# vedant-jumle/reinforcement-learning-101

Hardware: AMD Instinct MI355X
Metric: env-steps/sec (whole node), N parallel drones, 1/2/4/8 MI355X; HBM GB/s %peak (higher is better)
Workload: dtype f64

## Files before the change

reinforcement-learning-101_amd/csrc/frame.h:

```cpp
#pragma once

#include <hip/hip_runtime.h>
#include <stdint.h>
#include <string.h>

#include <type_traits>

#include "dronestep.h"
#include "philox.h"
#include "trig.h"

#include "libm_tables.h"
__device__ const double dd_libm_pow_tab[384] = DD_LIBM_POW_TAB;
__device__ const uint64_t dd_libm_exp_tab[256] = DD_LIBM_EXP_TAB;
__device__ const double dd_libm_sincos_tab[440] = DD_LIBM_SINCOS_TAB;
#define DD_LIBM_FN __device__ __forceinline__
#define DD_LIBM_OPAQUE
#define DD_LIBM_ENTRY __device__ __forceinline__
#include "libm_ref.h"
#undef DD_LIBM_FN
#undef DD_LIBM_ENTRY
#undef DD_LIBM_SINCOS_FN
#undef DD_LIBM_OPAQUE

namespace dd {

constexpr double kDeg2Rad = 3.14159265358979323846 / 180.0;

template <bool kExact = false, bool kSgpr = false>
__device__ __forceinline__ void sincos_deg(double deg, double* s, double* c) {
    if constexpr (kExact) {
        libm::sincos(deg * kDeg2Rad, s, c);
        return;
    }
    trig::sincos<kSgpr>(deg * kDeg2Rad, s, c);
}

constexpr DDConfig reference_config() {
    DDConfig c{};
    c.gravity = 0.3;
    c.drag = 0.99;
    c.angular_drag = 0.95;
    c.main_thrust_power = 0.6;
    c.side_thrust_power = 0.3;
    c.fuel_main = 2.0;
    c.fuel_side = 1.0;
    c.max_fuel = 1000.0;
    c.drone_half_height = 20 / 2.0;
    c.dt = 1.0;
    c.platform_half_width = 100 / 2.0;
    c.platform_half_height = 20 / 2.0;
    c.platform_speed = 1.0;
    c.platform_min_x = 100 / 2;
    c.platform_max_x = 800 - 100 / 2;
    c.max_landing_velocity = 3.0;
    c.max_landing_angle = 20.0;
    c.world_width = 800;
    c.world_height = 600;
    c.oob_margin = 50;
    c.ground_level = 600 - 50;
    c.wind_x = 0.0;
    c.wind_y = 0.0;
    c.reward_step = -0.1;
    c.reward_landing = 100.0;
    c.reward_crash = -100.0;
    c.reward_out_of_fuel = -50.0;
    c.reward_out_of_bounds = -50.0;
    c.shaping_offset = 500;
    c.shaping_scale = 5000;
    c.vel_scale = 10.0;
    c.angle_scale = 180.0;
    c.drone_start_x = 800 / 2;
    c.drone_start_y = 100;
    c.drone_x_min = 100;
    c.drone_x_max = 700;
    c.drone_y_min = 50;
    c.drone_y_max = 250;
    c.platform_start_x = 800 / 2;
    c.platform_start_y = 600 - 100;
    c.platform_x_lo = 100 / 2 + 50;
    c.platform_x_hi = 800 - 100 / 2 - 50;
    c.platform_y_lo = 100;
    c.platform_y_hi = 550;
    c.wind_enabled = 0;
    c.platform_moving = 0;
    c.randomize_drone = 0;
    c.randomize_platform = 1;
    c.auto_reset = 0;
    c.seed = 0;
    return c;
}

struct Consts {
    DDConfig c;
    double inv_w, inv_h, inv_vel, inv_angle, inv_fuel, inv_shaping;
};

constexpr Consts make_consts(const DDConfig& c) {
    Consts k{};
    k.c = c;
    k.inv_w = 1.0 / c.world_width;
    k.inv_h = 1.0 / c.world_height;
    k.inv_vel = 1.0 / c.vel_scale;
    k.inv_angle = 1.0 / c.angle_scale;
    k.inv_fuel = 1.0 / c.max_fuel;
    k.inv_shaping = 1.0 / c.shaping_scale;
    return k;
}

__device__ constexpr Consts kRefConsts = make_consts(reference_config());

inline bool uses_reference_physics(const DDConfig& c) {
    if (c.wind_enabled || c.platform_moving) return false;
    const DDConfig r = reference_config();
    const double* a = &c.gravity;
    const double* b = &r.gravity;
    const int n = (int)((&c.angle_scale - &c.gravity) + 1);
    for (int j = 0; j < n; ++j) {
        if (a + j == &c.wind_x || a + j == &c.wind_y) continue;
        if (memcmp(a + j, b + j, sizeof(double)) != 0) return false;
    }
    return true;
}

__device__ __forceinline__ int32_t draw_range(uint32_t r, int32_t lo, uint32_t span) {
    return lo + (int32_t)(((uint64_t)r * span) >> 32);
}

struct Lane {
    double x, y, vx, vy, angle, omega, fuel, px, py, total;
    double speed, dist;
    uint32_t status;
    int32_t steps, episode;
};

template <bool kUnscaled = false>
__device__ __forceinline__ double measure(Lane& s) {
    const double dx = s.px - s.x, dy = s.py - s.y;
    const double ss = s.vx * s.vx + s.vy * s.vy;
    const double dd = dx * dx + dy * dy;
    if (!kUnscaled) {
        s.speed = sqrt(ss);
        s.dist = sqrt(dd);
        return ss;
    }
    if (__builtin_expect(__ballot(!(ss >= 0x1p-767) | !(dd >= 0x1p-767)) != 0, 0)) {
        s.speed = sqrt(ss);
        s.dist = sqrt(dd);
    } else {
        s.speed = trig::sqrt_unscaled(ss);
        s.dist = trig::sqrt_unscaled(dd);
    }
    return ss;
}

__device__ __forceinline__ void spawn_words(const DDConfig& c, int64_t env, int32_t episode, uint32_t (&r)[4]) {
    philox4x32_7((uint32_t)env, (uint32_t)((uint64_t)env >> 32), (uint32_t)episode, 0u, (uint32_t)c.seed,
                  (uint32_t)(c.seed >> 32), r);
}

template <bool kRandom = false>
__device__ __forceinline__ void spawn_from(const DDConfig& c, double max_fuel, const uint32_t (&r)[4], Lane& s) {
    if (kRandom || c.randomize_drone) {
        s.x = draw_range(r[0], c.drone_x_min, (uint32_t)(c.drone_x_max - c.drone_x_min + 1));
        s.y = draw_range(r[1], c.drone_y_min, (uint32_t)(c.drone_y_max - c.drone_y_min + 1));
    } else {
        s.x = c.drone_start_x;
        s.y = c.drone_start_y;
    }
    if (kRandom || c.randomize_platform) {
        s.px = draw_range(r[2], c.platform_x_lo, (uint32_t)(c.platform_x_hi - c.platform_x_lo));
        s.py = draw_range(r[3], c.platform_y_lo, (uint32_t)(c.platform_y_hi - c.platform_y_lo));
    } else {
        s.px = c.platform_start_x;
        s.py = c.platform_start_y;
    }
    s.vx = 0.0; s.vy = 0.0; s.angle = 0.0; s.omega = 0.0;
    s.fuel = max_fuel;
    s.status = 0u;
    s.steps = 0;
    s.total = 0.0;
    const double dx = s.px - s.x, dy = s.py - s.y;
    s.speed = 0.0;
    s.dist = trig::sqrt_unscaled(dx * dx + dy * dy);
}

template <bool kRandom = false>
__device__ __forceinline__ void spawn(const DDConfig& c, double max_fuel, int64_t env, Lane& s) {
    s.episode += 1;
    uint32_t r[4];
    spawn_words(c, env, s.episode, r);
    spawn_from<kRandom>(c, max_fuel, r, s);
}

struct SpawnAhead {
    uint32_t r[4];
    int32_t ep;
    static constexpr int kRefill = 32;

    __device__ __forceinline__ void init(const DDConfig& c, int64_t env, int32_t episode) {
        ep = episode + 1;
        spawn_words(c, env, ep, r);
    }
    __device__ __forceinline__ void refill(const DDConfig& c, int64_t env, int32_t episode, int f) {
        if ((f & (kRefill - 1)) == kRefill - 1) {
            const bool spent = ep != episode + 1;
            if (__ballot(spent)) {
                if (spent) init(c, env, episode);
            }
        }
    }
    __device__ __forceinline__ void respawn(const DDConfig& c, double max_fuel, int64_t env, Lane& s) {
        s.episode += 1;
        uint32_t w[4] = {r[0], r[1], r[2], r[3]};
        if (ep != s.episode) spawn_words(c, env, s.episode, w);
        spawn_from(c, max_fuel, w, s);
    }
};

__device__ __forceinline__ double wrap_angle(double a) {
    double w = a > 180.0 ? a - 360.0 : a;
    w = a < -180.0 ? a + 360.0 : w;
    if (__builtin_expect(fabs(a) > 540.0, 0)) {
        w = trig::normalize_angle(a);
    }
    return w;
}

struct ThrustTrig {
    double s, c;
};
__device__ __forceinline__ void next_trig(const Lane& s, ThrustTrig& t) { sincos_deg<false>(s.angle, &t.s, &t.c); }

template <bool kRef, bool kFlat, bool kExact = false, bool kDefer = false, bool kPipe = false>
__device__ __forceinline__ double frame(const Consts& k, const DDConfig& sw, uint32_t act, Lane& s, bool* risky_out,
                                        const ThrustTrig* tt = nullptr) {
    static_assert(!kPipe || (kFlat && !kExact), "the pipelined thrust trig is the loops' fast frame");
    static_assert(!kDefer || (kRef && kFlat && !kExact), "deferred frames: reference world, rollout form");
    const DDConfig& c = k.c;

    const double ty = -c.main_thrust_power;
    constexpr bool kSgpr = !kFlat;
    const auto thrust = [&](double sa, double ca, double* dvx, double* dvy) __attribute__((always_inline)) {
        if constexpr (kRef) {
            *dvx = c.main_thrust_power * sa + 0.0;
            *dvy = ty * ca;
        } else {
            *dvx = 0.0 * ca - ty * sa;
            *dvy = 0.0 * sa + ty * ca;
        }
    };
    const bool main_on = (act & 1u) && s.fuel > 0.0;
    if constexpr (kFlat) {
        double sa, ca, dvx, dvy;
        if constexpr (kPipe) {
            sa = tt->s;
            ca = tt->c;
        } else {
            sincos_deg<kExact>(s.angle, &sa, &ca);
        }
        thrust(sa, ca, &dvx, &dvy);
        s.vx = main_on ? s.vx + dvx : s.vx;
        s.vy = main_on ? s.vy + dvy : s.vy;
        s.fuel = main_on ? s.fuel - c.fuel_main : s.fuel;
        const bool left_on = (act & 2u) && s.fuel > 0.0;
        s.omega = left_on ? s.omega - c.side_thrust_power : s.omega;
        s.fuel = left_on ? s.fuel - c.fuel_side : s.fuel;
        const bool right_on = (act & 4u) && s.fuel > 0.0;
        s.omega = right_on ? s.omega + c.side_thrust_power : s.omega;
        s.fuel = right_on ? s.fuel - c.fuel_side : s.fuel;
    } else {
        if (main_on) {
            double sa, ca, dvx, dvy;
            sincos_deg<kExact, kSgpr>(s.angle, &sa, &ca);
            thrust(sa, ca, &dvx, &dvy);
            s.vx += dvx;
            s.vy += dvy;
            s.fuel -= c.fuel_main;
        }
        if ((act & 2u) && s.fuel > 0.0) { s.omega -= c.side_thrust_power; s.fuel -= c.fuel_side; }
        if ((act & 4u) && s.fuel > 0.0) { s.omega += c.side_thrust_power; s.fuel -= c.fuel_side; }
    }
    s.fuel = s.fuel > 0.0 ? s.fuel : 0.0;

    if (!kRef && sw.wind_enabled) { s.vx += sw.wind_x; s.vy += sw.wind_y; }

    s.vy += c.gravity * c.dt;
    s.vx *= c.drag;
    s.vy *= c.drag;
    s.x += s.vx * c.dt;
    s.y += s.vy * c.dt;
    s.angle += s.omega * c.dt;
    s.omega *= c.angular_drag;
    s.angle = kFlat ? wrap_angle(s.angle) : trig::normalize_angle(s.angle);

    if (!kRef && sw.platform_moving) {
        const double dir = (s.status & DD_ST_PLAT_LEFT) ? -1.0 : 1.0;
        s.px += c.platform_speed * dir * c.dt;
        if (s.px <= c.platform_min_x) { s.px = c.platform_min_x; s.status &= ~DD_ST_PLAT_LEFT; }
        else if (s.px >= c.platform_max_x) { s.px = c.platform_max_x; s.status |= DD_ST_PLAT_LEFT; }
    }

    const auto close = [](double q, double b) { return fabs(q - b) <= 0x1p-20 * (1.0 + fabs(b)); };
    bool risky = false;
    if constexpr (!kExact) {
        if constexpr (kRef) {
            constexpr DDConfig r = reference_config();
            static_assert(-r.oob_margin == -50 && r.world_width + r.oob_margin == 850 && r.ground_level == 550,
                          "float boundary constants");
            const float xf = (float)s.x, yf = (float)s.y;
            const float qx = fabsf(fabsf(xf - 400.0f) - 450.0f), qy = fabsf(fabsf(yf - 250.0f) - 300.0f);
            risky = fminf(qx, qy) == 0.0f;
        } else {
            const bool q0 = close(s.y, c.ground_level), q1 = close(s.x, -c.oob_margin),
                       q2 = close(s.x, c.world_width + c.oob_margin), q3 = close(s.y, -c.oob_margin),
                       q4 = close(s.y, c.world_height + c.oob_margin);
            risky = q0 | q1 | q2 | q3 | q4;
        }
    }

    const double ss = kDefer ? s.vx * s.vx + s.vy * s.vy : measure<!kFlat>(s);
    const bool upright = fabs(s.angle) <= c.max_landing_angle;
    bool on_pad = false;
    const double rx = c.platform_half_width + fabs(c.drone_half_height);
    const double ry = c.platform_half_height + fabs(c.drone_half_height);
    const bool near_pad = upright && fma(-fabs(s.x), 0x1p-30, fabs(s.x - s.px)) <= rx + 1.0 &&
                          fma(-fabs(s.y), 0x1p-30, fabs(s.y - s.py)) <= ry + 1.0;
    if constexpr (kRef && !kExact) {
        const bool edge = fabs(ss - 9.0) <= 0x1p-20;
        static_assert(reference_config().max_landing_velocity == 3.0, "the squared speed limit");
        const bool slow = kDefer ? !(ss > 9.0) : !(s.speed > c.max_landing_velocity);
        risky |= near_pad & edge;
        const bool pad_test = near_pad & slow;
        if ((kFlat && !kDefer) || pad_test) {
            static_assert(reference_config().max_landing_angle == 20.0 &&
                              reference_config().drone_half_height == 10.0 &&
                              reference_config().platform_half_width == 50.0 &&
                              reference_config().platform_half_height == 10.0,
                          "sincos_upright_deg's range; the pad's half extents");
            double sb, cb;
            trig::sincos_upright_deg<kSgpr>(s.angle, &sb, &cb);
            const double bx = s.x - c.drone_half_height * sb;
            const double by = s.y + c.drone_half_height * cb;
            const double dxp = bx - s.px, dyp = by - s.py;
            const bool in_x = fabs(dxp) <= c.platform_half_width, in_y = fabs(dyp) <= c.platform_half_height;
            const bool in_box = in_x & in_y;
            const double m = fmin(fabs(fabs(dxp) - c.platform_half_width), fabs(fabs(dyp) - c.platform_half_height));
            const bool band = m <= 0x1p-19 * (1.0 + fabs(bx) + fabs(by));
            on_pad = pad_test && in_box;
            risky |= pad_test && band;
        }
    } else if (near_pad) {
        const bool edge = kRef ? fabs(ss - 9.0) <= 0x1p-20 : close(s.speed, c.max_landing_velocity);
        bool slow = !(s.speed > c.max_landing_velocity);
        if constexpr (kExact) {
            if (edge) {
                double sq = 0.0, v = s.vx;
#pragma unroll 1
                for (int q = 0; q < 2; ++q) {
                    sq += libm::pow2(v);
                    v = s.vy;
                }
                slow = !(sqrt(sq) > c.max_landing_velocity);
            }
        } else {
            risky |= edge;
        }
        if (slow) {
            double sb, cb;
            sincos_deg<kExact, kSgpr>(s.angle, &sb, &cb);
            const double bx = s.x + (0.0 * cb - c.drone_half_height * sb);
            const double by = s.y + (0.0 * sb + c.drone_half_height * cb);
            on_pad = (s.px - c.platform_half_width <= bx) & (bx <= s.px + c.platform_half_width) &
                     (s.py - c.platform_half_height <= by) & (by <= s.py + c.platform_half_height);
            if constexpr (!kExact) {
                const double m = fmin(fmin(fabs(bx - (s.px - c.platform_half_width)),
                                           fabs(bx - (s.px + c.platform_half_width))),
                                      fmin(fabs(by - (s.py - c.platform_half_height)),
                                           fabs(by - (s.py + c.platform_half_height))));
                risky |= m <= 0x1p-19 * (1.0 + fabs(bx) + fabs(by));
            }
        }
    }
    if constexpr (!kExact) *risky_out = risky;

    const bool landing = on_pad;
    const bool crash = s.y > c.ground_level;
    const bool no_fuel = s.fuel <= 0.0;
    const bool oob = (s.x < -c.oob_margin) | (s.x > c.world_width + c.oob_margin) |
                     (s.y < -c.oob_margin) | (s.y > c.world_height + c.oob_margin);
    double term = trig::div_exact(c.shaping_offset - s.dist, c.shaping_scale, k.inv_shaping);
    const bool terminal = landing | crash | no_fuel | oob;
    if constexpr (kRef) {
        constexpr DDConfig r = reference_config();
        static_assert(r.reward_landing == 100.0 && r.reward_crash == -100.0 && r.reward_out_of_fuel == -50.0 &&
                      r.reward_out_of_bounds == -50.0, "integer terminal rewards");
        const int32_t ti = landing ? 100 : crash ? -100 : -50;
        term = terminal ? (double)ti : term;
    } else {
        term = oob ? c.reward_out_of_bounds : term;
        term = no_fuel ? c.reward_out_of_fuel : term;
        term = crash ? c.reward_crash : term;
        term = landing ? c.reward_landing : term;
    }
    s.status |= landing ? (DD_ST_LANDED | DD_ST_DONE) : terminal ? (DD_ST_CRASHED | DD_ST_DONE) : 0u;
    if constexpr (kDefer) {
        s.steps += 1;
        return 0.0;
    }
    const double reward = c.reward_step + term;
    s.total += reward;
    s.steps += 1;
    return reward;
}



template <typename T>
__device__ __forceinline__ double finish_deferred(Lane& s, bool was_done, bool auto_reset, double& total) {
    constexpr DDConfig r = reference_config();
    const double dx = s.px - s.x, dy = s.py - s.y;
    s.speed = sqrt(s.vx * s.vx + s.vy * s.vy);
    s.dist = sqrt(dx * dx + dy * dy);
    if (was_done) {
        total = auto_reset ? 0.0 : total;
        return 0.0;
    }
    const bool terminal = (s.status & DD_ST_DONE) != 0;
    const int32_t ti = (s.status & DD_ST_LANDED) ? 100 : s.y > r.ground_level ? -100 : -50;
    double term = trig::div_exact(r.shaping_offset - s.dist, r.shaping_scale, kRefConsts.inv_shaping);
    term = terminal ? (double)ti : term;
    const double reward = r.reward_step + term;
    total = (double)(T)(total + reward);
    return reward;
}

template <bool kRef, bool kFlat, bool kDefer = false, bool kPipe = false, typename TQ = double>
__device__ __forceinline__ double frame_checked(const Consts& k, const DDConfig& sw, uint32_t act, Lane& s,
                                                ThrustTrig* tt = nullptr) {
    const Lane s0 = s;
    bool risky = false;
    double reward = frame<kRef, kFlat, false, kDefer, kPipe>(k, sw, act, s, &risky, tt);
    if constexpr (kPipe) sincos_deg<false>((double)(TQ)s.angle, &tt->s, &tt->c);
    if (__builtin_expect(__ballot(risky) != 0, 0)) {
        if (risky) {
            s = s0;
            reward = frame<kRef, false, true>(k, sw, act, s, nullptr);
        }
    }
    return reward;
}

template <bool kGuard = false, bool kExactDiv = false>
__device__ __forceinline__ void observe_values(const Consts& k, const Lane& s, double v[13]) {
    const DDConfig& c = k.c;
    const double dx = s.px - s.x, dy = s.py - s.y;
#define DD_Q(x, d, inv) \
    (!kExactDiv ? (x) * (inv) : kGuard ? trig::div_exact_guarded((x), (d), (inv)) : trig::div_exact((x), (d), (inv)))
    v[0] = DD_Q(s.x, c.world_width, k.inv_w);
    v[1] = DD_Q(s.y, c.world_height, k.inv_h);
    v[2] = DD_Q(s.vx, c.vel_scale, k.inv_vel);
    v[3] = DD_Q(s.vy, c.vel_scale, k.inv_vel);
    v[4] = DD_Q(s.angle, c.angle_scale, k.inv_angle);
    v[5] = DD_Q(s.omega, c.vel_scale, k.inv_vel);
    v[6] = DD_Q(s.fuel, c.max_fuel, k.inv_fuel);
    v[7] = DD_Q(s.px, c.world_width, k.inv_w);
    v[8] = DD_Q(s.py, c.world_height, k.inv_h);
    v[9] = DD_Q(s.dist, c.world_width, k.inv_w);
    v[10] = DD_Q(dx, c.world_width, k.inv_w);
    v[11] = DD_Q(dy, c.world_height, k.inv_h);
    v[12] = DD_Q(s.speed, c.vel_scale, k.inv_vel);
#undef DD_Q
}

__device__ __forceinline__ void write_obs_row(const double v[13], uint32_t status, float* o) {
#pragma unroll
    for (int j = 0; j < 13; ++j) o[j] = (float)v[j];
    o[13] = (status & DD_ST_LANDED) ? 1.0f : 0.0f;
    o[14] = (status & DD_ST_CRASHED) ? 1.0f : 0.0f;
}

template <bool kGuard = false>
__device__ __forceinline__ void observe(const Consts& k, const Lane& s, float* o) {
    double v[13];
    observe_values<kGuard>(k, s, v);
    write_obs_row(v, s.status, o);
}

enum { kShapeNone = 0, kShapePpo = 1, kShapeReinforce = 2 };

__device__ __forceinline__ double notebook_reward(const double v[13], uint32_t status, double prev_dist) {
    const double vx = v[2], vy = v[3], angle = v[4], fuel = v[6], dist = v[9], dx = v[10], dy = v[11],
                 speed = v[12];
    const bool have_prev = !__builtin_isnan(prev_dist);
    const double delta = prev_dist - dist;
    const double vtp = dist > 1e-6 ? (vx * dx + vy * dy) / dist : 0.0;
    const bool fast_toward = (speed >= 0.15) & (vtp > 0.1) & (dist > 0.065);
    const double clipped = fmin(fmax(delta * 1000 * (1.0 + speed * 2.0), -2.0), 5.0);
    const bool away = !fast_toward & (delta < -0.001);
    double distance = fast_toward ? clipped : away ? -2.0 * fabs(delta) * 1000 : 0.0;
    double hovering = (fast_toward | away) ? 0.0 : speed < 0.05 ? -1.0 : speed < 0.15 ? -0.3 : 0.0;
    distance = have_prev ? distance : 0.0;
    hovering = have_prev ? hovering : 0.0;
    double total = 0.0;
    total += -0.5;
    total += distance;
    total += hovering;
    const double excess = fabs(angle) - (((0.20 - 0.111) * dist) + 0.111);
    total += -(excess > 0.0 ? excess : 0.0);
    const double over = dist < 1 ? speed - 0.1 : speed - 0.6;
    total += (dist < 1 ? -2.0 : -1.0) * (over > 0.0 ? over : 0.0);
    total += dy > 0.0 ? 0.0 : dy * 4.0;
    const bool landed = status & DD_ST_LANDED, crashed = status & DD_ST_CRASHED;
    const double crash_term = dist > 0.3 ? -200.0 - 100.0 : -200.0;
    total += landed ? 800.0 + fuel * 100.0 : crashed ? crash_term : 0.0;
    return total;
}

__device__ __forceinline__ double reinforce_reward(const double v[13], uint32_t status) {
    const double vx = v[2], vy = v[3], angle = v[4], fuel = v[6], dist = v[9], dx = v[10], dy = v[11],
                 speed = v[12];
    constexpr double kScale = 1.0 - 0.3;
    const double time_penalty = -(kScale * (1.0 / (1.0 + (50.0 * (dist * dist))))) - 0.3;
    const double odx0 = -dx, ody0 = -dy;
    const double onorm = sqrt(odx0 * odx0 + ody0 * ody0);
    const double odx = odx0 / onorm, ody = ody0 / onorm;
    const double align_v = (vx / speed) * odx + (vy / speed) * ody;
    const double align = onorm < 1e-6 ? 1.0 : speed < 1e-6 ? 0.0 : align_v;
    const bool above = (dist > 0.065) & (dy > 0.0);
    const double sig = 4.5 * (1.0 / (1.0 + exp(10.0 * (dist - 0.5))));
    const double distance = above ? ((align > 0.0 ? 1.0 : 0.0) * speed) * sig : 0.0;
    const double valign = (above & (align > 0.0)) ? 0.5 : 0.0;
    double total = time_penalty;
    total += distance;
    total += valign;
    const double excess = fabs(angle) - (((0.20 - 0.111) * dist) + 0.111);
    total += -(excess > 0.0 ? excess : 0.0);
    const double over = dist < 1 ? speed - 0.1 : speed - 0.4;
    total += (dist < 1 ? -2.0 : -1.0) * (over > 0.0 ? over : 0.0);
    total += dy > 0.0 ? 0.0 : dy * 4.0;
    const bool landed = status & DD_ST_LANDED, crashed = status & DD_ST_CRASHED;
    const double crash_term = dist > 0.3 ? -200.0 - 100.0 : -200.0;
    total += landed ? 500.0 + fuel * 100.0 : crashed ? crash_term : 0.0;
    return total;
}

__device__ __forceinline__ void notebook_reward_parts(const double v[13], uint32_t status, double prev_dist,
                                                      double parts[8]) {
    const double vx = v[2], vy = v[3], angle = v[4], fuel = v[6], dist = v[9], dx = v[10], dy = v[11],
                 speed = v[12];
    parts[0] = -(1.0 * (1.0 / (1.0 + (100.0 * (dist * dist))))) - 0.0;
    const bool have_prev = !__builtin_isnan(prev_dist);
    const double delta = prev_dist - dist;
    const double vtp = dist > 1e-6 ? (vx * dx + vy * dy) / dist : 0.0;
    const bool fast_toward = (speed >= 0.15) & (vtp > 0.1) & (dist > 0.065);
    const double clipped = fmin(fmax(delta * 1000 * (1.0 + speed * 2.0), -2.0), 5.0);
    const bool away = !fast_toward & (delta < -0.001);
    double distance = fast_toward ? clipped : away ? -2.0 * fabs(delta) * 1000 : 0.0;
    double hovering = (fast_toward | away) ? 0.0 : speed < 0.05 ? -1.0 : speed < 0.15 ? -0.3 : 0.0;
    parts[1] = have_prev ? distance : 0.0;
    parts[2] = have_prev ? hovering : 0.0;
    const double excess = fabs(angle) - (((0.20 - 0.111) * dist) + 0.111);
    parts[3] = -(excess > 0.0 ? excess : 0.0);
    const double over = dist < 1 ? speed - 0.1 : speed - 0.6;
    parts[4] = (dist < 1 ? -2.0 : -1.0) * (over > 0.0 ? over : 0.0);
    parts[5] = dy > 0.0 ? 0.0 : dy * 4.0;
    const bool landed = status & DD_ST_LANDED, crashed = status & DD_ST_CRASHED;
    const double crash_term = dist > 0.3 ? -200.0 - 100.0 : -200.0;
    parts[6] = landed ? 800.0 + fuel * 100.0 : crashed ? crash_term : 0.0;
    double total = 0.0;
    total += -0.5;
#pragma unroll
    for (int j = 1; j < 7; ++j) total += parts[j];
    parts[7] = total;
}

__device__ __forceinline__ void reinforce_reward_parts(const double v[13], uint32_t status, double parts[8]) {
    const double vx = v[2], vy = v[3], angle = v[4], fuel = v[6], dist = v[9], dx = v[10], dy = v[11],
                 speed = v[12];
    constexpr double kScale = 1.0 - 0.3;
    parts[0] = -(kScale * (1.0 / (1.0 + (50.0 * (dist * dist))))) - 0.3;
    const double odx0 = -dx, ody0 = -dy;
    const double onorm = sqrt(odx0 * odx0 + ody0 * ody0);
    const double odx = odx0 / onorm, ody = ody0 / onorm;
    const double align_v = (vx / speed) * odx + (vy / speed) * ody;
    const double align = onorm < 1e-6 ? 1.0 : speed < 1e-6 ? 0.0 : align_v;
    const bool above = (dist > 0.065) & (dy > 0.0);
    const double sig = 4.5 * (1.0 / (1.0 + exp(10.0 * (dist - 0.5))));
    parts[1] = above ? ((align > 0.0 ? 1.0 : 0.0) * speed) * sig : 0.0;
    parts[2] = (above & (align > 0.0)) ? 0.5 : 0.0;
    const double excess = fabs(angle) - (((0.20 - 0.111) * dist) + 0.111);
    parts[3] = -(excess > 0.0 ? excess : 0.0);
    const double over = dist < 1 ? speed - 0.1 : speed - 0.4;
    parts[4] = (dist < 1 ? -2.0 : -1.0) * (over > 0.0 ? over : 0.0);
    parts[5] = dy > 0.0 ? 0.0 : dy * 4.0;
    const bool landed = status & DD_ST_LANDED, crashed = status & DD_ST_CRASHED;
    const double crash_term = dist > 0.3 ? -200.0 - 100.0 : -200.0;
    parts[6] = landed ? 500.0 + fuel * 100.0 : crashed ? crash_term : 0.0;
    double total = parts[0];
#pragma unroll
    for (int j = 1; j < 7; ++j) total += parts[j];
    parts[7] = total;
}

template <typename T, bool kRef = false>
__device__ __forceinline__ void quantize(Lane& s) {
    s.x = (T)s.x; s.y = (T)s.y; s.vx = (T)s.vx; s.vy = (T)s.vy; s.angle = (T)s.angle;
    s.omega = (T)s.omega; s.fuel = (T)s.fuel; s.total = (T)s.total;
    if constexpr (!kRef) { s.px = (T)s.px; s.py = (T)s.py; }
}

}
```

reinforcement-learning-101_amd/csrc/step_fast.hip:

```cpp

#include <hip/hip_runtime.h>
#include <stdint.h>

#include "dronestep.h"
#include "step_tile.h"

namespace dd {

constexpr bool kFastLoadsEpisode = true;

template <typename T>
__global__ __launch_bounds__(kStepBlock) void step_fast_kernel(StepArgs p, Soa<T> a) {
    step_tile<T, DD_ACT_BITMASK, true, kShapeNone, false, true, kFastLoadsEpisode>(p, a, a);
}

template <typename T>
void launch_step_fast(const StepArgs& p, const Soa<T>& a, hipStream_t s) {
    const unsigned blocks = (unsigned)(p.n / kStepBlock);
    hipLaunchKernelGGL((step_fast_kernel<T>), dim3(blocks), dim3(kStepBlock), 0, s, p, a);
}

template void launch_step_fast<float>(const StepArgs&, const Soa<float>&, hipStream_t);
template void launch_step_fast<double>(const StepArgs&, const Soa<double>&, hipStream_t);

}
```

reinforcement-learning-101_amd/csrc/step_tile.h:

```cpp
#pragma once

#include <hip/hip_runtime.h>
#include <stdint.h>

#include "dronestep.h"
#include "frame.h"
#include "lane_io.h"
#include "launch.h"
#include "trig.h"

namespace dd {

struct StepArgs {
    Consts k;
    const void* actions;
    void* reward;
    uint8_t* done;
    float* obs;
    int32_t* done_idx;
    int32_t* done_count;
    int32_t n;
    int32_t idx_base;
    double* shaped_hist;
    int64_t hist_stride;
    void* shaped_reward;
    uint8_t* shaped_done;
    int32_t max_steps;
};

constexpr int kStepBlock = 256;

template <typename T>
struct Raw {
    T x, y, vx, vy, angle, omega, fuel, px, py, total;
    uint32_t status, act;
    int32_t steps, episode;
};

template <typename T, int AFMT, bool kEpisode = false>
__device__ __forceinline__ void load_raw(const Soa<T>& a, const void* actions, uint32_t i, Raw<T>& r) {
    r.act = load_action<AFMT>(actions, i);
    r.x = at(a.x, i); r.y = at(a.y, i); r.vx = at(a.vx, i); r.vy = at(a.vy, i);
    r.angle = at(a.angle, i); r.omega = at(a.omega, i); r.fuel = at(a.fuel, i);
    r.px = at(a.px, i); r.py = at(a.py, i); r.total = at(a.total, i);
    r.status = at(a.status, i);
    r.steps = at(a.steps, i);
    if constexpr (kEpisode) r.episode = at(a.episode, i);
    asm volatile("" ::"v"(r.act));
}

template <typename T, bool kRef, int kShape, bool kPP, bool kFast = false, bool kEpisode = false>
__device__ __forceinline__ bool finish_lane(const StepArgs& p, const Soa<T>& a, const Soa<T>& o, uint32_t i,
                                            const Raw<T>& r, float* orow) {
    static_assert(!kFast || (kRef && kShape == kShapeNone && !kPP), "the headline shape: kRef, engine reward, in place");
    static_assert(!kEpisode || kFast, "only the headline kernel loads episode with the state");
    const DDConfig& sw = p.k.c;
    const Consts& k = kRef ? kRefConsts : p.k;
    Lane s;
    s.x = r.x; s.y = r.y; s.vx = r.vx; s.vy = r.vy; s.angle = r.angle; s.omega = r.omega;
    s.fuel = r.fuel; s.px = r.px; s.py = r.py; s.total = r.total;
    s.status = r.status;
    s.steps = r.steps;
    bool ended = false;
    bool respawned = false;
    double reward;
    double shaped = 0.0;
    bool shaped_done = false;
    if (s.status & DD_ST_DONE) {
        reward = 0.0;
        if (kFast || sw.auto_reset) {
            if constexpr (kEpisode) s.episode = r.episode;
            else s.episode = at(a.episode, i);
            spawn<kFast>(sw, k.c.max_fuel, a.env_id_base + i, s);
            respawned = true;
            if constexpr (kShape == kShapePpo) {
                at(p.shaped_hist, i) = trig::div_exact(s.dist, k.c.world_width, k.inv_w);
                at(p.shaped_hist + p.hist_stride, i) = __builtin_nan("");
            }
        } else {
            measure(s);
            shaped_done = true;
        }
    } else {
        bool rk = false;
        reward = frame<kRef, false>(k, sw, r.act, s, &rk);
        if (__builtin_expect(__ballot(rk) != 0, 0)) {
            if (rk) {
                s.x = r.x; s.y = r.y; s.vx = r.vx; s.vy = r.vy; s.angle = r.angle; s.omega = r.omega;
                s.fuel = r.fuel; s.px = r.px; s.py = r.py; s.total = r.total; s.status = r.status;
                s.steps = r.steps;
                reward = frame<kRef, false, true>(k, sw, r.act, s, nullptr);
            }
        }
        if constexpr (kShape != kShapeNone) {
            double v[13];
            observe_values<false, true>(k, s, v);
            if constexpr (kShape == kShapePpo) {
                double* slot = p.shaped_hist + (s.steps & 1) * p.hist_stride;
                shaped = notebook_reward(v, s.status, at(slot, i));
                at(slot, i) = v[9];
            } else {
                shaped = reinforce_reward(v, s.status);
            }
            shaped_done = (s.status & DD_ST_DONE) != 0;
            if (p.max_steps > 0 && s.steps >= p.max_steps) {
                shaped = (s.status & DD_ST_LANDED) ? shaped : shaped - 500;
                shaped_done = true;
                s.status |= DD_ST_DONE;
            }
            if (kFast || p.obs) observe(k, s, orow);
        }
        ended = (s.status & DD_ST_DONE) != 0;
    }
    const bool sticky = !kFast && (r.status & DD_ST_DONE) && !respawned && !kPP;
    if (!sticky) {
        uint32_t j = i;
        asm volatile("" : "+v"(j));
        store_dynamics(o, j, s);
        put_state(o.steps, j, s.steps);
        put_state(o.total, j, (T)s.total);
        const bool moving = !kRef && sw.platform_moving;
        if (moving || respawned) put_state(a.px, j, (T)s.px);
        if (moving || ended || respawned) put_state(a.status, j, (uint8_t)s.status);
        if (respawned) { put_state(a.py, j, (T)s.py); put_state(a.episode, j, s.episode); }
    }
    put_out(static_cast<T*>(p.reward), i, (T)reward);
    put_out(p.done, i, (uint8_t)((s.status & DD_ST_DONE) ? 1 : 0));
    if constexpr (kShape != kShapeNone) {
        put_out(static_cast<T*>(p.shaped_reward), i, (T)shaped);
        put_out(p.shaped_done, i, (uint8_t)(shaped_done ? 1 : 0));
        if ((kFast || p.obs) && ((r.status & DD_ST_DONE) != 0)) observe(k, s, orow);
    } else {
        if (kFast || p.obs) observe(k, s, orow);
    }
    return ended;
}

template <typename T, int AFMT, bool kRef, int kShape, bool kPP, bool kFast = false, bool kEpisode = false>
__device__ __forceinline__ void step_tile(const StepArgs& p, const Soa<T>& a, const Soa<T>& o) {
    __shared__ __attribute__((aligned(16))) float tile[kStepBlock * DD_OBS_DIM];
    const uint32_t row0 = blockIdx.x * kStepBlock;
    const uint32_t i = row0 + threadIdx.x;
    asm volatile("" ::"s"(a.x), "s"(a.y), "s"(a.vx), "s"(a.vy), "s"(a.angle), "s"(a.omega), "s"(a.fuel),
                 "s"(a.px), "s"(a.py), "s"(a.total), "s"(a.status), "s"(a.steps), "s"(p.actions));
    Raw<T> r;
    if (kFast || i < (uint32_t)p.n) load_raw<T, AFMT, kEpisode>(a, p.actions, i, r);
    const bool ended = (kFast || i < (uint32_t)p.n) &&
                       finish_lane<T, kRef, kShape, kPP, kFast, kEpisode>(p, a, o, i, r, tile + threadIdx.x * DD_OBS_DIM);
    if (!kFast && p.done_idx) {
        const uint64_t m = __ballot(ended);
        if (m) {
            const int lane = threadIdx.x & (kWave - 1);
            const int leader = __ffsll((unsigned long long)m) - 1;
            const int before = __builtin_amdgcn_mbcnt_hi((uint32_t)(m >> 32),
                                                         __builtin_amdgcn_mbcnt_lo((uint32_t)m, 0));
            int b = 0;
            if (lane == leader) b = atomicAdd(p.done_count, __popcll(m));
            b = __shfl(b, leader);
            if (ended) p.done_idx[b + before] = p.idx_base + (int32_t)i;
        }
    }
    if (kFast || p.obs) {
        const uint32_t wrow0 = row0 + (threadIdx.x & ~(kWave - 1));
        const float* wtile = tile + (threadIdx.x & ~(kWave - 1)) * DD_OBS_DIM;
        float* dst = p.obs + (size_t)wrow0 * DD_OBS_DIM;
        if (kFast || (wrow0 + kWave <= (uint32_t)p.n && (reinterpret_cast<uintptr_t>(p.obs) & 15u) == 0)) {
            flush_obs_wave_full(wtile, dst);
        } else {
            const int rows = (int)min((int64_t)kWave, max((int64_t)0, (int64_t)p.n - wrow0));
            flush_obs_wave(wtile, dst, rows);
        }
    }
}

enum { kStepGeneric = 0, kStepFast = 1 };

constexpr int64_t kStepFastMaxLanes = int64_t(1) << 18;

inline int step_variant_of(const DDConfig& c, const DDStepIO& io, int shape, bool ref, int64_t first, int64_t len) {
    if (!ref || shape != kShapeNone || io.action_format != DD_ACT_BITMASK) return kStepGeneric;
    if (io.state_out || io.done_idx || io.shaped_hist || io.shaped_reward || io.shaped_done) return kStepGeneric;
    if (!c.auto_reset || !c.randomize_drone || !c.randomize_platform) return kStepGeneric;
    if (!io.obs || (reinterpret_cast<uintptr_t>(io.obs + first * DD_OBS_DIM) & 15u) != 0) return kStepGeneric;
    if (len <= 0 || len % kStepBlock != 0 || len > kStepFastMaxLanes) return kStepGeneric;
    return kStepFast;
}

template <typename T>
void launch_step_fast(const StepArgs& p, const Soa<T>& a, hipStream_t s);

}
```

Measured before the change: 39.23 billion.

## Hoist respawn Philox draws before state loads land and cap waves per EU

Result: no change. 39.39 billion, median of 2 (+0.4%).

```diff
diff --git a/reinforcement-learning-101_amd/csrc/frame.h b/reinforcement-learning-101_amd/csrc/frame.h
--- a/reinforcement-learning-101_amd/csrc/frame.h
+++ b/reinforcement-learning-101_amd/csrc/frame.h
@@ -159,6 +159,17 @@
                   (uint32_t)(c.seed >> 32), r);
 }
 
+__device__ __forceinline__ void spawn_rest(double max_fuel, Lane& s) {
+    s.vx = 0.0; s.vy = 0.0; s.angle = 0.0; s.omega = 0.0;
+    s.fuel = max_fuel;
+    s.status = 0u;
+    s.steps = 0;
+    s.total = 0.0;
+    const double dx = s.px - s.x, dy = s.py - s.y;
+    s.speed = 0.0;
+    s.dist = trig::sqrt_unscaled(dx * dx + dy * dy);
+}
+
 template <bool kRandom = false>
 __device__ __forceinline__ void spawn_from(const DDConfig& c, double max_fuel, const uint32_t (&r)[4], Lane& s) {
     if (kRandom || c.randomize_drone) {
@@ -175,14 +186,23 @@
         s.px = c.platform_start_x;
         s.py = c.platform_start_y;
     }
-    s.vx = 0.0; s.vy = 0.0; s.angle = 0.0; s.omega = 0.0;
-    s.fuel = max_fuel;
-    s.status = 0u;
-    s.steps = 0;
-    s.total = 0.0;
-    const double dx = s.px - s.x, dy = s.py - s.y;
-    s.speed = 0.0;
-    s.dist = trig::sqrt_unscaled(dx * dx + dy * dy);
+    spawn_rest(max_fuel, s);
+}
+
+struct SpawnPos {
+    int32_t x, y, px, py;
+};
+
+template <bool kRandom = false>
+__device__ __forceinline__ void spawn_draws(const DDConfig& c, const uint32_t (&r)[4], SpawnPos& q) {
+    Lane t;
+    spawn_from<kRandom>(c, 0.0, r, t);
+    q.x = (int32_t)t.x; q.y = (int32_t)t.y; q.px = (int32_t)t.px; q.py = (int32_t)t.py;
+}
+
+__device__ __forceinline__ void spawn_assemble(double max_fuel, const SpawnPos& q, Lane& s) {
+    s.x = q.x; s.y = q.y; s.px = q.px; s.py = q.py;
+    spawn_rest(max_fuel, s);
 }
 
 template <bool kRandom = false>
diff --git a/reinforcement-learning-101_amd/csrc/step_fast.hip b/reinforcement-learning-101_amd/csrc/step_fast.hip
--- a/reinforcement-learning-101_amd/csrc/step_fast.hip
+++ b/reinforcement-learning-101_amd/csrc/step_fast.hip
@@ -10,7 +10,8 @@
 constexpr bool kFastLoadsEpisode = true;
 
 template <typename T>
-__global__ __launch_bounds__(kStepBlock) void step_fast_kernel(StepArgs p, Soa<T> a) {
+__global__ __launch_bounds__(kStepBlock) __attribute__((amdgpu_waves_per_eu(5))) void step_fast_kernel(StepArgs p,
+                                                                                                        Soa<T> a) {
     step_tile<T, DD_ACT_BITMASK, true, kShapeNone, false, true, kFastLoadsEpisode>(p, a, a);
 }
 
diff --git a/reinforcement-learning-101_amd/csrc/step_tile.h b/reinforcement-learning-101_amd/csrc/step_tile.h
--- a/reinforcement-learning-101_amd/csrc/step_tile.h
+++ b/reinforcement-learning-101_amd/csrc/step_tile.h
@@ -39,14 +39,29 @@
 
 template <typename T, int AFMT, bool kEpisode = false>
 __device__ __forceinline__ void load_raw(const Soa<T>& a, const void* actions, uint32_t i, Raw<T>& r) {
+    if constexpr (kEpisode) { r.status = at(a.status, i); r.episode = at(a.episode, i); }
     r.act = load_action<AFMT>(actions, i);
     r.x = at(a.x, i); r.y = at(a.y, i); r.vx = at(a.vx, i); r.vy = at(a.vy, i);
     r.angle = at(a.angle, i); r.omega = at(a.omega, i); r.fuel = at(a.fuel, i);
     r.px = at(a.px, i); r.py = at(a.py, i); r.total = at(a.total, i);
-    r.status = at(a.status, i);
+    if constexpr (!kEpisode) r.status = at(a.status, i);
     r.steps = at(a.steps, i);
-    if constexpr (kEpisode) r.episode = at(a.episode, i);
-    asm volatile("" ::"v"(r.act));
+    if constexpr (kEpisode) asm volatile("" ::"v"(r.status));
+    else asm volatile("" ::"v"(r.act));
+}
+
+template <typename T>
+__device__ __forceinline__ void early_spawn(const DDConfig& sw, int64_t env, const Raw<T>& r, SpawnPos& q) {
+    q.x = 0; q.y = 0; q.px = 0; q.py = 0;
+    const bool done = (r.status & DD_ST_DONE) != 0;
+    if (__ballot(done) != 0) {
+        if (done) {
+            uint32_t w[4];
+            spawn_words(sw, env, r.episode + 1, w);
+            spawn_draws<true>(sw, w, q);
+        }
+    }
+    asm volatile("" : "+v"(q.x), "+v"(q.y), "+v"(q.px), "+v"(q.py));
 }
 
 template <typename T, bool kRef, int kShape, bool kPP, bool kFast = false, bool kEpisode = false>
@@ -56,6 +71,8 @@
     static_assert(!kEpisode || kFast, "only the headline kernel loads episode with the state");
     const DDConfig& sw = p.k.c;
     const Consts& k = kRef ? kRefConsts : p.k;
+    SpawnPos drawn;
+    if constexpr (kEpisode) early_spawn(sw, a.env_id_base + i, r, drawn);
     Lane s;
     s.x = r.x; s.y = r.y; s.vx = r.vx; s.vy = r.vy; s.angle = r.angle; s.omega = r.omega;
     s.fuel = r.fuel; s.px = r.px; s.py = r.py; s.total = r.total;
@@ -69,9 +86,13 @@
     if (s.status & DD_ST_DONE) {
         reward = 0.0;
         if (kFast || sw.auto_reset) {
-            if constexpr (kEpisode) s.episode = r.episode;
-            else s.episode = at(a.episode, i);
-            spawn<kFast>(sw, k.c.max_fuel, a.env_id_base + i, s);
+            if constexpr (kEpisode) {
+                s.episode = r.episode + 1;
+                spawn_assemble(k.c.max_fuel, drawn, s);
+            } else {
+                s.episode = at(a.episode, i);
+                spawn<kFast>(sw, k.c.max_fuel, a.env_id_base + i, s);
+            }
             respawned = true;
             if constexpr (kShape == kShapePpo) {
                 at(p.shaped_hist, i) = trig::div_exact(s.dist, k.c.world_width, k.inv_w);
@@ -143,6 +164,11 @@
     const uint32_t i = row0 + threadIdx.x;
     asm volatile("" ::"s"(a.x), "s"(a.y), "s"(a.vx), "s"(a.vy), "s"(a.angle), "s"(a.omega), "s"(a.fuel),
                  "s"(a.px), "s"(a.py), "s"(a.total), "s"(a.status), "s"(a.steps), "s"(p.actions));
+    if constexpr (kEpisode) {
+        const DDConfig& c = p.k.c;
+        asm volatile("" ::"s"(c.seed), "s"(c.drone_x_min), "s"(c.drone_x_max), "s"(c.drone_y_min), "s"(c.drone_y_max),
+                     "s"(c.platform_x_lo), "s"(c.platform_x_hi), "s"(c.platform_y_lo), "s"(c.platform_y_hi));
+    }
     Raw<T> r;
     if (kFast || i < (uint32_t)p.n) load_raw<T, AFMT, kEpisode>(a, p.actions, i, r);
     const bool ended = (kFast || i < (uint32_t)p.n) &&
```
